# SysCV/LiDAR_snow_sim

Hardware: AMD Instinct MI355X
Metric: augmented points/s/GPU (64x2048 sweep, 2.5 mm/h); HBM roofline % -- value: rows resident in HBM when the clock starts (device-resident API: augment_batch on CUDA tensors); with H2D of the rows and D2H of the results inside the clock: value_pcie_inclusive (higher is better)
Workload: dtype f64

## Files before the change

### lidar_snow_sim_amd/csrc/sg_beam.h

```cpp
#pragma once
#include "sg_math.h"
#include "sg_atan_cr.h"
#include "sg_range_index.h"

#if defined(__HIP_DEVICE_COMPILE__)
#define SG_GLOBAL __attribute__((address_space(1)))
#else
#define SG_GLOBAL
#endif
template <typename P> __device__ __forceinline__ const SG_GLOBAL P *sg_gptr(const P *p) { return (const SG_GLOBAL P *)p; }

#if defined(__HIP_DEVICE_COMPILE__)
template <int CTRL, int ROW_MASK> __device__ __forceinline__ int sg_dpp(int old, int v) { return __builtin_amdgcn_update_dpp(old, v, CTRL, ROW_MASK, 0xf, false); }
__device__ __forceinline__ int sg_wave_incl_add(int v)
{
    v += sg_dpp<0x111, 0xf>(0, v); v += sg_dpp<0x112, 0xf>(0, v); v += sg_dpp<0x114, 0xf>(0, v); v += sg_dpp<0x118, 0xf>(0, v);
    v += sg_dpp<0x142, 0xa>(0, v);
    v += sg_dpp<0x143, 0xc>(0, v);
    return v;
}
__device__ __forceinline__ int sg_wave_incl_max(int v)
{
    constexpr int I = (int)0x80000000;
    v = max(v, sg_dpp<0x111, 0xf>(I, v)); v = max(v, sg_dpp<0x112, 0xf>(I, v)); v = max(v, sg_dpp<0x114, 0xf>(I, v)); v = max(v, sg_dpp<0x118, 0xf>(I, v));
// ... 261 lines not shown
typedef unsigned int SgTailRaw __attribute__((ext_vector_type(4)));
__device__ __forceinline__ SgTailRaw sg_tail_load(const SG_GLOBAL SgEntry *fp) { return *reinterpret_cast<const SG_GLOBAL SgTailRaw *>(&fp->rho); }
__device__ __forceinline__ SgTail sg_tail_pin(SgTailRaw v)
{
    asm volatile("" : "+v"(v));
    SgTail t; t.rho = __hiloint2double((int)v.y, (int)v.x); t.flags = v.z;
    return t;
}
#else
typedef SgTail SgTailRaw;
__device__ __forceinline__ SgTailRaw sg_tail_load(const SgEntry *fp) { SgTail t; t.rho = fp->rho; t.flags = fp->flags; return t; }
__device__ __forceinline__ SgTail sg_tail_pin(SgTailRaw v) { return v; }
#endif

__device__ __forceinline__ uint32_t sg_hit_word(uint32_t e, bool hit_r, bool hit_l)
{
    return e | (hit_r ? 0x40000000u : 0u) | (hit_l ? 0x80000000u : 0u);
}
__device__ __forceinline__ void sg_hit_angles(uint32_t w, const SgEntry *__restrict__ entries, double theta_r, double theta_l, double &a1, double &a2)
{
    const SG_GLOBAL SgEntry *f = sg_gptr(entries) + (w & 0x3fffffffu);
    a1 = (w & 0x40000000u) ? theta_r : f->t0;
    a2 = (w & 0x80000000u) ? theta_l : f->t1;
}

template <int N>
__device__ __forceinline__ void sg_hit_angles_all(const uint32_t (&w)[N], int L, const SgEntry *__restrict__ entries, double theta_r, double theta_l,
                                                  double (&a1)[N], double (&a2)[N])
{
#if defined(__HIP_DEVICE_COMPILE__)
    SgTailRaw raw[N];
#pragma unroll
    for (int j = 0; j < N; ++j) {
        const SG_GLOBAL SgEntry *f = sg_gptr(entries) + (j < L ? (w[j] & 0x3fffffffu) : 0u);
        raw[j] = *reinterpret_cast<const SG_GLOBAL SgTailRaw *>(&f->t0);
    }
#pragma unroll
    for (int j = 0; j < N; ++j) {
        a1[j] = (w[j] & 0x40000000u) ? theta_r : __hiloint2double((int)raw[j].y, (int)raw[j].x);
        a2[j] = (w[j] & 0x80000000u) ? theta_l : __hiloint2double((int)raw[j].w, (int)raw[j].z);
    }
#else
    for (int j = 0; j < N; ++j) if (j < L) sg_hit_angles(w[j], entries, theta_r, theta_l, a1[j], a2[j]);
#endif
}

struct SgQsPair { uint32_t x, y; };
#if defined(__HIP_DEVICE_COMPILE__)
typedef unsigned int SgQsRaw __attribute__((ext_vector_type(2), aligned(4)));
__device__ __forceinline__ SgQsPair sg_qs_load(const SG_GLOBAL uint32_t *p)
{
    const SgQsRaw v = *reinterpret_cast<const SG_GLOBAL SgQsRaw *>(p);
    return SgQsPair{v.x, v.y};
}
#else
__device__ __forceinline__ SgQsPair sg_qs_load(const uint32_t *p) { return SgQsPair{p[0], p[1]}; }
#endif

template <typename T, int LMAX, int STRIDE, bool DEFER = false, bool COMPACT = false, bool UTAB = false>
__device__ __forceinline__ int sg_wave_scan_t(bool act, T px, T py, T pz, const SgTable tab, double beam_div_deg, double *s_a1, double *s_a2,
                                              double *s_rho, int *s_cnt, int *s_key, int *s_st, int tid, SgBeamOut &out, T &d_t, T &theta_t,
                                              bool EXACT_TAN, double *ov_blk = nullptr, int ov_cap = 0)
{
    out.overflow = 0; out.range_error = 0; out.diff2 = 0.0; out.has_power = 0; out.n_flakes = 0; out.n_hits = 0;
    out.label = 0; out.new_i = 0; out.k_best = 0;
    const int lane = tid & 63, wbase = tid & ~63;
    SgBeamGeo g{};
// ... 718 lines not shown
```

### lidar_snow_sim_amd/csrc/sg_common.h

```cpp
#pragma once
#include <stddef.h>
#include <stdint.h>

#define SG_PI 3.141592653589793
#define SG_TWO_PI (2 * SG_PI)
#define SG_RBINS 1230
#define SG_NBINS 2048
#define SG_BIN_MARGIN 1e-6
#define SG_BEAM_MARGIN 1e-9
#define SG_TBL_STRIDE 16
#define SG_BLKREC 8
#define SG_HITS_UNDECIDED 0x40000000
#define SG_MAX_LASERS 256
#define SG_LCAP 63
#define SG_TILE 1024

struct SgEntry {
    double phi;
    double x, y, r;
    double t0, t1;
    double rho;
    uint32_t flags;
    uint32_t src;
};
// ... 54 lines not shown
    const SgLasers *las;
    const double *rgrid;
    double beam_div_deg;
    uint32_t *rec;
    uint32_t *rec_q;
    void *rng;
    int32_t *status;
    int32_t *tier_hint;
    unsigned long long *diff2;
    int32_t exact_math;
    int32_t n_cls;
    int32_t cls_cap[SG_MAX_CLASSES];
    const int32_t *seg_blk;
    const int64_t *seg_start;
    const int32_t *seg_cnt;
    const int32_t *seg_frame;
    const int32_t *seg_n;
    const int32_t *seg_of_blk;
    int64_t grid_blocks;
    int32_t q_chunk;
    int64_t blk_lo, blk_hi;
    const int32_t *chunk_blk;
    int32_t chunk;
    double *dq;
    int32_t *dq_g;
    uint16_t *dq_sc;
    unsigned long long *qn;
    int2_t *pw_items;
    int32_t *pw_count;
    int2_t *pw_items1;
    int32_t front_max;
    int64_t n_regions_ub;
    int32_t blk_rows;
    int32_t kp_lds_quarters;
    int64_t dq_n;
    int32_t *tier_list;
    int32_t *tier_info;
    int64_t tier_stride;
    int32_t *tier_sparse;
    int32_t *tn, *tbase;
    int32_t cls;
    int32_t work_lo, work_hi;
    int32_t work_hint;
    int32_t *redo_list;
    int32_t *redo_cnt;
    double *tq;
    uint16_t *tq_sc;
// ... 126 lines not shown
```

### lidar_snow_sim_amd/csrc/sg_host.h

```cpp
#pragma once
#include <hip/hip_runtime.h>

#include <algorithm>
#include <array>
#include <cmath>
#include <cstdio>
#include <cstdlib>
#include <cstring>
#include <string>
#include <vector>

#include "../../include/snowgpu.h"
#include "sg_common.h"
#include "sg_prepass.h"
#include "sg_plane.h"
#include "sg_assemble.h"
#include "sg_device_args.h"

#pragma GCC visibility push(hidden)

struct DeviceTable {
    SgEntry *entries = nullptr;
    uint32_t *bin_start = nullptr;
    uint32_t *bin_q = nullptr;
// ... 59 lines not shown
    DevBuf<int32_t> fpss_tile, fpss_seg;
    DevBuf<uint32_t> ball_entry, ball_cell;
    DevBuf<uint8_t> ball_x, ball_y, ball_z;
    DevBuf<int32_t> ball_src;
    DevBuf<unsigned long long> range_key;
    DevBuf<uint32_t> nn_entry;
    DevBuf<int32_t> nn_box;
    DevBuf<uint8_t> nn_rec;
    DevBuf<double> box_rec;
    DevBuf<unsigned long long> box_table;
    DevBuf<double> roi_rec;
    DevBuf<unsigned long long> roi_table;
    DevBuf<int32_t> roi_runs;
    DevBuf<double> iou_rec;
    DevBuf<int32_t> nms_order, nms_cand;
    DevBuf<int32_t> tile_hist, tile_base, perm, ctile_cnt, ctile_base, table_ids, out_src;
    DevBuf<uint8_t> srows;
    DevBuf<int32_t> tile_unsorted, frame_unsorted;
    DevBuf<unsigned long long> seg_tbl_cnt, seg_tbl_base;
    DevBuf<int32_t> seg_blk, seg_cnt, seg_frame, seg_n, seg_of_blk;
    DevBuf<int64_t> seg_start;
    DevBuf<uint32_t> rec, rec_q;
    DevBuf<uint8_t> rng;
    DevBuf<double> dq;
    DevBuf<int32_t> dq_g;
    DevBuf<uint16_t> dq_sc;
    DevBuf<unsigned long long> qn;
    DevBuf<int2_t> pw_items;
    DevBuf<double> ov;
    DevBuf<uint16_t> ov_sc;
    DevBuf<int32_t> tier_list, tier_sparse, tbase, redo_list;
    DevBuf<double> tq[SG_MAX_CLASSES];
    DevBuf<uint16_t> tq_sc[SG_MAX_CLASSES];
    DevBuf<double> h_lists;
    int64_t tier_cap_override = 0;
    int first_tier_override = 0;
    int few = 2;
    int heavy_tail = -1;
    int tier_rows = -1;
    hipStream_t lane_stream[3] = {nullptr, nullptr, nullptr};
    int stats_early = -1;
    int prepass_with_few = -1;
    bool serial = false;
    DevBuf<int32_t> chunk_blk;
    DevBuf<uint16_t> rank;
    DevBuf<uint8_t> keep, rows_in, rows_out;
    DevBuf<int64_t> frame_off, out_counts, out_stats;
// ... 166 lines not shown
```

### lidar_snow_sim_amd/csrc/snowgpu_batch.cpp

```cpp
#include "sg_host.h"
#include "sg_launch.h"

static int sync_tables(snowgpu_ctx *ctx)
{
    if (!ctx->tables_dirty) return SNOWGPU_OK;
    const size_t n = std::max<size_t>(ctx->tables.size(), 1);
    if (n > ctx->d_tables_cap) {
        if (ctx->d_tables) { (void)hipStreamSynchronize(ctx->stream); (void)hipFree(ctx->d_tables); }
        HIPCHK(ctx, hipMalloc((void **)&ctx->d_tables, n * sizeof(SgTable)));
        ctx->d_tables_cap = n;
    }
    std::vector<SgTable> h(n);
    for (size_t i = 0; i < ctx->tables.size(); ++i) h[i] = ctx->tables[i].desc;
    HIPCHK(ctx, hipMemcpy(ctx->d_tables, h.data(), n * sizeof(SgTable), hipMemcpyHostToDevice));
    ctx->tables_dirty = false;
    return SNOWGPU_OK;
}

static void choose_tiers(const snowgpu_ctx *ctx, double beam_div_deg, int tiers[4], int *n_tiers)
{
    const double expect = (double)ctx->max_flakes * (beam_div_deg * (SG_PI / 180.0)) / SG_TWO_PI;
    int first = expect <= 24.0 ? 4 : (expect <= 48.0 ? 8 : (expect <= 96.0 ? 16 : SG_LCAP));
    if (ctx->first_tier_override == 4 || ctx->first_tier_override == 8 || ctx->first_tier_override == 16 ||
        ctx->first_tier_override == SG_LCAP)
// ... 190 lines not shown
    const int h_lanes = 256;
    const int h_cap = (int)std::min<uint32_t>(std::max<uint32_t>(R->max_flakes, 64u), 8192u);
    a.n_cls = n_cls;
    for (int k = 0; k + 1 < n_cls; ++k) a.cls_cap[k] = tiers[k + 1];
    a.cls_cap[n_cls - 1] = h_cap;
    ENSURE(ctx, ctx->h_lists, (size_t)4 * (size_t)(h_cap + 1) * (size_t)h_lanes);
    a.h_lists = ctx->h_lists.p; a.h_cap = h_cap; a.h_lanes = h_lanes;
    a.tier_list = ctx->tier_list.p; a.tier_stride = b.n_total; a.tier_sparse = ctx->tier_sparse.p;
    if (tier_rows) {
        ENSURE(ctx, ctx->redo_list, n * (size_t)n_tiers);
        a.redo_list = ctx->redo_list.p;
    }
    const bool use_ov = tiers[0] < SG_OV_CAP && n_cls >= 2 && !tier_rows &&
                        R->tier_cap_override <= 0 && n * SG_OV_STRIDE * sizeof(double) <= ((size_t)40 << 30);
    int64_t tq_caps[SG_MAX_CLASSES] = {0, 0, 0, 0};
    for (int k = 0; k + 1 < n_cls && !tier_rows; ++k) {
        if (use_ov && tiers[k + 1] <= SG_OV_CAP) continue;
        tq_caps[k] = tier_queue_cap(R, tiers[k + 1], b.n_total);
        ENSURE(ctx, ctx->tq[k], ((size_t)tq_caps[k] + 64) * (3 * (size_t)tiers[k + 1] + 2));
        ENSURE(ctx, ctx->tq_sc[k], (size_t)tq_caps[k]);
    }
    a.q_chunk = (int32_t)q_chunk;
    {
        const size_t planes = 3 * (size_t)tiers[0] + 2;
        if (n * planes * sizeof(double) > ((size_t)64 << 30))
            return fail(ctx, SNOWGPU_E_INVALID, "batch too large for the dict queue of this table density: split it");
        if (b.n_frames >= (1 << 22)) return fail(ctx, SNOWGPU_E_INVALID, "too many frames in one batch");
        ENSURE(ctx, ctx->dq, (n + 64) * planes);
        ENSURE(ctx, ctx->dq_g, n);
        ENSURE(ctx, ctx->dq_sc, n);
        if (!seg_small) HIPCHK(ctx, hipMemsetAsync(ctx->qn.p, 0, sizeof(unsigned long long) * zero_words, st));
        a.tn = (int32_t *)(ctx->qn.p + regions); a.tbase = ctx->tbase.p;
        a.diff2 = ctx->qn.p + 3 * regions;
        int32_t *small = (int32_t *)(ctx->qn.p + 3 * regions + (size_t)b.n_frames);
        a.tier_info = small; a.pw_count = small + 8; a.redo_cnt = small + 12;
        a.dq = ctx->dq.p; a.dq_g = ctx->dq_g.p; a.dq_sc = ctx->dq_sc.p; a.qn = ctx->qn.p; a.dq_n = b.n_total;
        const int lanes = first_block < 64 ? first_block : 64;
        a.n_regions_ub = use_seg ? (int64_t)b.n_frames * 256 : (b.n_total + a.q_chunk - 1) / a.q_chunk;
        a.blk_rows = first_block;
        a.kp_lds_quarters = 2;
        const size_t items_cap = n / (size_t)lanes + 2 * (size_t)a.n_regions_ub + 64;
        ENSURE(ctx, ctx->pw_items, 2 * items_cap);
        a.pw_items = ctx->pw_items.p;
        a.pw_items1 = (R->few > 0 && !b.dbg_count && lanes == 64) ? ctx->pw_items.p + items_cap : nullptr;
        a.front_max = a.pw_items1 ? std::min(R->few, std::min(3, tiers[0])) : 1;
    }
    if (use_ov) {
        ENSURE(ctx, ctx->ov, (n + 256) * SG_OV_STRIDE);
        ENSURE(ctx, ctx->ov_sc, n + 256);
        a.ov = ctx->ov.p; a.ov_sc = ctx->ov_sc.p; a.ov_cap = SG_OV_CAP;
    }
// ... 171 lines not shown
```

### lidar_snow_sim_amd/csrc/snowgpu_kernels.hip

```cpp
#include <hip/hip_runtime.h>
#include <algorithm>
#include "sg_beam.h"
#include "sg_few.h"
#include "sg_kutil.h"
#include "sg_launch.h"

#ifndef SG_NB4
#define SG_NB4 4
#endif
#ifndef SG_KP_WIN
#define SG_KP_WIN 3
#endif
#ifndef SG_FP_WAVES
#define SG_FP_WAVES 6
#endif
#ifndef SG_FP_WAVES_SEG
#define SG_FP_WAVES_SEG 7
#endif
#ifndef SG_NB_TIERS
#define SG_NB_TIERS 4
#endif
#ifndef SG_KP_THREE_MAX
#define SG_KP_THREE_MAX 16
#endif
#ifndef SG_KP_THREE_MIN
#define SG_KP_THREE_MIN 8
// ... 205 lines not shown
            } else {
                tier_k = k;
                pending = true;
            }
        } else if (o.range_error) {
            atomicCAS(&a.status[0], 0, 4 );
            atomicCAS(&a.status[1], -1, (int32_t)g);
        }
    }
    if constexpr (!LIST) {
        if (__ballot(tier_k >= 0)) {
            for (int k = 0; k < a.n_cls; ++k) {
                const unsigned long long m = __ballot(tier_k == k);
                if (!m) continue;
                const int leader = __ffsll((long long)m) - 1;
                int base = 0;
                if ((tid & 63) == leader) base = atomicAdd(&a.tn[(int64_t)__builtin_amdgcn_readfirstlane(region) * SG_MAX_CLASSES + k], (int)__popcll(m));
                base = __shfl(base, leader);
                if (tier_k == k) a.tier_sparse[(int64_t)k * a.tier_stride + q_base + base + (int)__popcll(m & sg_lanemask_lt())] = (int32_t)g;
            }
        }
    }
    if constexpr (DICT) {
        constexpr int P = SG_QPLANES(LMAX);
        auto hand_over = [&](double *q, int64_t slot) {
            q[sg_qaddr<P>(slot, 0)] = (double)d_t;
            q[sg_qaddr<P>(slot, 1)] = (double)theta_t;
            double th_r, th_l;
            sg_beam_limits((double)theta_t, a.beam_div_deg, th_r, th_l);
            if constexpr (LMAX <= 4) {
                double x1[LMAX], x2[LMAX];
                uint32_t hw[LMAX];
#pragma unroll
                for (int j = 0; j < LMAX; ++j) hw[j] = reinterpret_cast<const uint32_t *>(s_a1)[j * BLOCK + tid];
                sg_hit_angles_all<LMAX>(hw, L, tab.entries, th_r, th_l, x1, x2);
#pragma unroll
                for (int j = 0; j < LMAX; ++j)
                    if (j < L) {
                        q[sg_qaddr<P>(slot, 2 + 3 * j)] = x1[j];
                        q[sg_qaddr<P>(slot, 3 + 3 * j)] = x2[j];
                        q[sg_qaddr<P>(slot, 4 + 3 * j)] = s_rho[j * BLOCK + tid];
                    }
            } else {
                for (int j = 0; j < L; ++j) {
                    double x1, x2;
                    sg_hit_angles(reinterpret_cast<const uint32_t *>(s_a1)[j * BLOCK + tid], tab.entries, th_r, th_l, x1, x2);
                    q[sg_qaddr<P>(slot, 2 + 3 * j)] = x1;
                    q[sg_qaddr<P>(slot, 3 + 3 * j)] = x2;
                    q[sg_qaddr<P>(slot, 4 + 3 * j)] = s_rho[j * BLOCK + tid];
                }
            }
        };
        const bool front = o.has_power && L <= a.front_max, back = o.has_power && L > a.front_max;
        const unsigned long long mf = __ballot(front), mb = __ballot(back);
        if (mf | mb) {
            const int leader = __ffsll((long long)(mf | mb)) - 1;
            unsigned long long base = 0;
            if ((tid & 63) == leader)
                base = atomicAdd(&a.qn[__builtin_amdgcn_readfirstlane(region)], (unsigned long long)__popcll(mf) | ((unsigned long long)__popcll(mb) << 32));
            const unsigned blo = __shfl((unsigned)(base & 0xffffffffull), leader), bhi = __shfl((unsigned)(base >> 32), leader);
            if (o.has_power) {
                const int64_t slot = front ? q_base + (int)blo + (int)__popcll(mf & sg_lanemask_lt())
                                           : q_base + q_size - 1 - ((int)bhi + (int)__popcll(mb & sg_lanemask_lt()));
                hand_over(a.dq, slot);
                a.dq_g[slot] = (int32_t)g;
                a.dq_sc[slot] = (uint16_t)(L | (ch << 8));
                rec = SG_REC_SLOT | (uint32_t)slot;
            }
        }
    } else {
        constexpr int NB = LMAX <= 4 ? 4 : 8;
        if (o.has_power) {
            double best = 0.0;
// ... 138 lines not shown
    }
    for (int k = 0; k < nb; k += lanes_back)
        a.pw_items[base++] = make_int2((int)(q_base + q_size - nb + k), (nb - k < lanes_back ? nb - k : lanes_back) | (f1 << 10));
}

__global__ __launch_bounds__(256) void k_tier_gather(SgBeamArgs a, int n_regions_ub)
{
    const int r = blockIdx.x * 4 + (int)(threadIdx.x >> 6), lane = (int)(threadIdx.x & 63);
    if (blockIdx.x == 0 && threadIdx.x < SG_MAX_CLASSES) a.status[2 + threadIdx.x] = a.tier_info[threadIdx.x];
    if (blockIdx.x == 0 && threadIdx.x < SG_MAX_CLASSES && a.tier_hint) a.tier_hint[threadIdx.x] = a.tier_info[threadIdx.x];
    if (blockIdx.x == 0 && threadIdx.x == 0 && a.tier_hint) a.tier_hint[SG_MAX_CLASSES] = (int32_t)((a.n_total >> 10) + 1);
    int q_size = 0, f1 = 0;
    int64_t q_base = 0;
    if (!sg_region(a, r, n_regions_ub, q_base, q_size, f1)) return;
    for (int k = 0; k < a.n_cls; ++k) {
        const int c = a.tn[(int64_t)r * SG_MAX_CLASSES + k];
        if (c == 0) continue;
        const int32_t *src = a.tier_sparse + (int64_t)k * a.tier_stride + q_base;
        int32_t *dst = a.tier_list + (int64_t)k * a.tier_stride + a.tbase[(int64_t)r * SG_MAX_CLASSES + k];
        for (int i = lane; i < c; i += 64) dst[i] = src[i];
    }
}

template <typename T, int LMAX, int BLOCK, bool LISTQ>
__device__ __forceinline__ void sg_kp_item(const SgBeamArgs &a, char *smem, const int ov_list, const int64_t work_off,
                                           const int start, const int cnt, const int item_f)
{
    constexpr int LANES = BLOCK < 64 ? BLOCK : 64;
    constexpr int WIN = BLOCK < 64 ? 1 : SG_KP_WIN;
    constexpr int P = SG_QPLANES(LMAX);
    double *s_a1 = (double *)smem;
    constexpr bool THREE = SG_KP_THREE_MAX > 0 && LMAX <= SG_KP_THREE_MAX && LMAX >= SG_KP_THREE_MIN;
    double *s_a2 = s_a1 + (LMAX + 1) * BLOCK;
    double *s_rho = s_a2 + (LMAX + 1) * BLOCK;
    double *s_ratio = THREE ? s_rho : s_rho + (LMAX + 1) * BLOCK;
    double *s_work = THREE ? s_a2 : s_ratio;
    const int tid = threadIdx.x, lane = tid & 63;
    const int ltid = BLOCK < 64 ? lane : tid;
    const double *planes = LISTQ ? a.tq : a.dq;
    const uint16_t *scs = LISTQ ? a.tq_sc : a.dq_sc;
    static_assert(WIN <= 4, "the window's permutation passes through one 64-double row segment of the wave");
    uint16_t *s_perm = (uint16_t *)(s_ratio + (BLOCK < 64 ? 0 : (tid & ~63)));
    int perm[WIN];
    const bool sorted = WIN > 1 && cnt > LANES;
    if constexpr (WIN > 1) {
        if (sorted) {
            int key[WIN], rank[WIN];
            int64_t at[WIN];
            unsigned scw[WIN];
#pragma unroll
            for (int r = 0; r < WIN; ++r) { const int idx = r * 64 + lane; at[r] = (int64_t)start + (idx < cnt ? idx : 0); }
            if (LISTQ && ov_list) {
#pragma unroll
                for (int r = 0; r < WIN; ++r) at[r] = (int64_t)a.tier_list[work_off + at[r]];
#pragma unroll
                for (int r = 0; r < WIN; ++r) scw[r] = (unsigned)a.ov_sc[at[r]];
            } else {
#pragma unroll
                for (int r = 0; r < WIN; ++r) scw[r] = (unsigned)scs[at[r]];
            }
#pragma unroll
            for (int r = 0; r < WIN; ++r) {
// ... 15 lines not shown
            place(254); place(255);
#pragma unroll
            for (int r = 0; r < WIN; ++r) s_perm[rank[r]] = (uint16_t)(r * 64 + lane);
            asm volatile("s_waitcnt lgkmcnt(0)" ::: "memory");
#pragma unroll
            for (int r = 0; r < WIN; ++r) perm[r] = s_perm[r * 64 + lane];
            asm volatile("s_waitcnt lgkmcnt(0)" ::: "memory");
        }
    }
    const int rounds = (cnt + LANES - 1) / LANES;
    for (int r = 0; r < rounds; ++r) {
        const int idx = r * LANES + lane;
        const bool in = lane < LANES && idx < cnt;
        int pos = idx;
        if constexpr (WIN > 1) {
            if (sorted) {
#pragma unroll
                for (int q = 0; q < WIN; ++q) if (q == r) pos = perm[q];
            }
        }
        const int64_t slot = (int64_t)start + pos;
        unsigned sc = 0xffffu;
        int32_t g = 0;
        double d = 0.0, tc = 0.0, f_a1 = 0.0, f_a2 = 0.0, f_rho = 0.0;
        const double *qb = planes;
        int qs = 64;
        if (in) {
            g = LISTQ ? a.tier_list[work_off + slot] : a.dq_g[slot];
            if (LISTQ && ov_list) { qb = a.ov + (size_t)g * SG_OV_STRIDE; qs = 1; sc = a.ov_sc[g]; }
            else { qb = planes + sg_qaddr<P>(slot, 0); sc = scs[slot]; }
            d = qb[0];
            tc = qb[qs];
            f_a1 = qb[2 * qs]; f_a2 = qb[3 * qs]; f_rho = qb[4 * qs];
        }
        const bool live = in && sc != 0xffffu;
        const int L = (int)(sc & 255u), ch = (int)(sc >> 8);
        int f = 0;
        SgBeamOut o;
        o.overflow = 0; o.range_error = 0; o.diff2 = 0.0; o.has_power = 0; o.n_flakes = 0; o.n_hits = 0; o.label = 0; o.new_i = 0; o.k_best = 0;
        constexpr int NB = LMAX <= 4 ? SG_NB4 : SG_NB_TIERS;
        int S = 0, nw = 0, k_best = 0;
        double best = 0.0;
        if (live) {
            f = item_f >= 0 ? item_f : sg_frame_of(a, g);
            unsigned long long ord = 0xfedcba9876543210ull;
            if (LISTQ) {
                s_a1[ltid] = f_a1; s_a2[ltid] = f_a2; s_rho[ltid] = f_rho;
                if constexpr (THREE) ord = 0;
                for (int h0 = 1; h0 < L; h0 += 8) {
                    double xa[8], xb[8], xr[8];
#pragma unroll
                    for (int c = 0; c < 8; ++c) {
                        const int h = h0 + c < L ? h0 + c : 0;
                        xa[c] = qb[(2 + 3 * h) * qs]; xb[c] = qb[(3 + 3 * h) * qs]; xr[c] = qb[(4 + 3 * h) * qs];
                    }
#pragma unroll
                    for (int c = 0; c < 8; ++c)
                        if (h0 + c < L) { s_a1[(h0 + c) * BLOCK + ltid] = xa[c]; s_a2[(h0 + c) * BLOCK + ltid] = xb[c]; s_rho[(h0 + c) * BLOCK + ltid] = xr[c]; }
                }
                for (int h = 1; h < L; ++h) {
                    const double x1 = s_a1[h * BLOCK + ltid], x2 = s_a2[h * BLOCK + ltid], r = s_rho[h * BLOCK + ltid];
                    int q = h;
                    while (q > 0 && (s_rho[(q - 1) * BLOCK + ltid] > r ||
                                     (s_rho[(q - 1) * BLOCK + ltid] == r && ov_list &&
                                      (s_a1[(q - 1) * BLOCK + ltid] > x1 || (s_a1[(q - 1) * BLOCK + ltid] == x1 && s_a2[(q - 1) * BLOCK + ltid] > x2))))) {
                        s_rho[q * BLOCK + ltid] = s_rho[(q - 1) * BLOCK + ltid]; s_a1[q * BLOCK + ltid] = s_a1[(q - 1) * BLOCK + ltid];
                        s_a2[q * BLOCK + ltid] = s_a2[(q - 1) * BLOCK + ltid];
                        --q;
                    }
                    if (q != h) { s_rho[q * BLOCK + ltid] = r; s_a1[q * BLOCK + ltid] = x1; s_a2[q * BLOCK + ltid] = x2; }
                    if constexpr (THREE) {
                        const unsigned long long low = (1ull << (4 * q)) - 1ull;
                        ord = (ord & low) | ((unsigned long long)h << (4 * q)) | ((ord & ~low) << 4);
                    }
                }
            } else {
                s_a1[ltid] = f_a1; s_a2[ltid] = f_a2;
                if constexpr (!THREE) s_rho[ltid] = f_rho;
                if constexpr (LMAX <= 4 && !THREE) {
                    double xa[LMAX - 1], xb[LMAX - 1], xr[LMAX - 1];
#pragma unroll
                    for (int j = 1; j < LMAX; ++j) { xa[j - 1] = qb[(2 + 3 * j) * qs]; xb[j - 1] = qb[(3 + 3 * j) * qs]; xr[j - 1] = qb[(4 + 3 * j) * qs]; }
#pragma unroll
                    for (int j = 1; j < LMAX; ++j)
                        if (j < L) { s_a1[j * BLOCK + ltid] = xa[j - 1]; s_a2[j * BLOCK + ltid] = xb[j - 1]; s_rho[j * BLOCK + ltid] = xr[j - 1]; }
                } else {
                    for (int j = 1; j < L; ++j) {
                        s_a1[j * BLOCK + ltid] = qb[(2 + 3 * j) * qs];
                        s_a2[j * BLOCK + ltid] = qb[(3 + 3 * j) * qs];
                        if constexpr (!THREE) s_rho[j * BLOCK + ltid] = qb[(4 + 3 * j) * qs];
                    }
                }
            }
            auto queue_rho = [&](int j) -> double {
                const int h = (int)((ord >> (4 * j)) & 15ull);
                return h == 0 ? f_rho : qb[(4 + 3 * h) * qs];
            };
            int32_t *dc = a.dbg_count ? a.dbg_count + g : nullptr;
            double *drj = a.dbg_count ? a.dbg_rj + (int64_t)g * a.dbg_cap : nullptr;
            double *dra = a.dbg_count ? a.dbg_ratio + (int64_t)g * a.dbg_cap : nullptr;
            unsigned long long srcmap = 0;
            if constexpr (THREE) S = sg_beam_dict<LMAX, BLOCK, false>(L, tc, d, a.beam_div_deg, s_a1, s_a2, nullptr, s_ratio, ltid, 0, nullptr, nullptr, nullptr, 0, &srcmap);
            else S = sg_beam_dict<LMAX, BLOCK>(L, tc, d, a.beam_div_deg, s_a1, s_a2, s_rho, s_ratio, ltid, a.dbg_cap, dc, drj, dra);
            if constexpr (THREE) {
                if (dc) {
                    *dc = S + 1;
                    for (int t = 0; t <= S && t < a.dbg_cap; ++t) {
                        const int j = (int)((srcmap >> (4 * t)) & 15ull);
                        drj[t] = t == S ? d : queue_rho(j);
                        dra[t] = s_ratio[t * BLOCK + ltid];
                    }
                }
            }
            if (S > 0) {
                const T d_t = (T)d;
                if constexpr (THREE) {
                    sg_beam_amp3<T, LMAX, BLOCK>(d_t, S, ch, a.las, s_a1, s_a2, s_rho, ltid, o,
                                                 [&](int t) { return queue_rho((int)((srcmap >> (4 * t)) & 15ull)); });
                } else sg_beam_amp<T, LMAX, BLOCK>(d_t, S, ch, a.las, s_a1, s_a2, s_rho, s_ratio, ltid, o, 0);
// ... 40 lines not shown
        if (work_n > a.work_hi) work_n = a.work_hi;
        work_off = (int64_t)a.cls * a.tier_stride;
        if (WIN > 1 && work_n <= (int64_t)step * LANES) item_slots = LANES;
        n_items = (int)((work_n + item_slots - 1) / item_slots);
    } else {
        n_items = *a.pw_count;
    }
    for (int i = (int)blockIdx.x * WAVES + __builtin_amdgcn_readfirstlane(tid >> 6); i < n_items; i += step) {
        int start, cnt, item_f = -1;
        if (LISTQ) {
            start = i * item_slots;
            cnt = (int)(work_n - start < item_slots ? work_n - start : item_slots);
        } else {
            const int2 d = a.pw_items[i];
            start = __builtin_amdgcn_readfirstlane(d.x);
            const int dy = __builtin_amdgcn_readfirstlane(d.y);
            cnt = dy & 1023; item_f = (dy >> 10) - 1;
        }
        sg_kp_item<T, LMAX, BLOCK, LISTQ>(a, smem, a.ov_list, work_off, start, cnt, item_f);
    }
}

template <typename T, int N>
__global__ __launch_bounds__(256, 4) void k_power_few(SgBeamArgs a, int qplanes)
{
    __shared__ double s_amp[N + 1][256], s_rho[N + 1][256], s_best[256];
    __shared__ int s_win[N + 1][256], s_zone[N + 1][256], s_k[256];
    __shared__ int s_mark[256];
    const int tid = (int)threadIdx.x, lane = tid & 63, wbase = tid & ~63;
    const int n_items = a.pw_count[1];
    const int step = (int)gridDim.x * 4;
    for (int i = (int)blockIdx.x * 4 + __builtin_amdgcn_readfirstlane(tid >> 6); i < n_items; i += step) {
        const int2 it = a.pw_items1[i];
        const int start = __builtin_amdgcn_readfirstlane(it.x), dy = __builtin_amdgcn_readfirstlane(it.y);
        const int cnt = dy & 1023, item_f = (dy >> 10) - 1;
        const bool live = lane < cnt;
        const int64_t slot = (int64_t)start + lane;
        SgBeamOut o;
        o.overflow = 0; o.range_error = 0; o.diff2 = 0.0; o.has_power = 0; o.n_flakes = 0; o.n_hits = 0; o.label = 0; o.new_i = 0; o.k_best = 0;
        int f = 0, ch = 0, S = 0, g = 0;
        SgFew<N> P{};
        int zone[N + 1], n = 0;
#pragma unroll
        for (int z = 0; z <= N; ++z) zone[z] = 0;
        if (live) {
            const double *q = a.dq + (slot >> 6) * (int64_t)(qplanes * 64) + (slot & 63);
            const unsigned sc = a.dq_sc[slot];
            const double d = q[0], tc = q[64];
            double a1[N], a2[N], rho[N];
#pragma unroll
            for (int j = 0; j < N; ++j) {
                a1[j] = q[(2 + 3 * j) * 64]; a2[j] = q[(3 + 3 * j) * 64]; rho[j] = q[(4 + 3 * j) * 64];
            }
            ch = (int)(sc >> 8);
            g = a.dq_g[slot];
            f = item_f >= 0 ? item_f : sg_frame_of(a, g);
            S = sg_few_prep<T, N>(d, tc, (int)(sc & 255u), a1, a2, rho, ch, a.las, a.beam_div_deg, P, o);
            if (S) {
                int ka, kb;
                sg_few_zone<N, 0>(P, 0.0, ka, kb);
                if (kb >= ka) { zone[0] = ka | ((kb - ka + 1) << 16); n += kb - ka + 1; }
                if constexpr (N >= 2) { sg_few_zone<N, 1>(P, 0.0, ka, kb); if (kb >= ka) { zone[1] = ka | ((kb - ka + 1) << 16); n += kb - ka + 1; } }
                if constexpr (N >= 3) { sg_few_zone<N, 2>(P, 0.0, ka, kb); if (kb >= ka) { zone[2] = ka | ((kb - ka + 1) << 16); n += kb - ka + 1; } }
                sg_few_zone<N, N>(P, 0.0, ka, kb);
                if (kb >= ka) { zone[N] = ka | ((kb - ka + 1) << 16); n += kb - ka + 1; }
            }
        }
#pragma unroll
        for (int t = 0; t < N; ++t) { s_amp[t][tid] = P.amp[t]; s_rho[t][tid] = P.rho[t]; s_win[t][tid] = P.k0[t] | (P.k1[t] << 16); }
        s_amp[N][tid] = P.tamp; s_rho[N][tid] = P.d; s_win[N][tid] = P.tk0 | (P.tk1 << 16);
#pragma unroll
        for (int z = 0; z <= N; ++z) s_zone[z][tid] = zone[z];
        s_best[tid] = 0.0; s_k[tid] = 0;
        asm volatile("" ::: "memory");
        const int incl = sg_wave_incl_add(n);
        const int excl = incl - n;
        const int total = __builtin_amdgcn_readlane(incl, 63);
        for (int base = 0; base < total; base += 64) {
            const int p = base + lane;
// ... 155 lines not shown
    constexpr int THREADS = BLOCK < 64 ? 64 : BLOCK, LANES = BLOCK < 64 ? BLOCK : 64;
    const int cus = sg_cu_count();
    unsigned per_cu = (unsigned)std::min<size_t>(32 * 64 / THREADS, std::max<size_t>(1, (size_t)(160 * 1024) / lds));
    if (!LISTQ && a->kp_lds_quarters > 0 && a->kp_lds_quarters < 4) per_cu = std::max(1u, per_cu * (unsigned)a->kp_lds_quarters / 4u);
    int64_t blocks = (int64_t)cus * per_cu;
    int64_t items_ub = LISTQ ? ((int64_t)a->work_hi + LANES - 1) / LANES : (a->n_total + LANES - 1) / LANES + 2 * a->n_regions_ub;
    if (LISTQ && a->work_hint > 0) items_ub = std::min<int64_t>(items_ub, (4 * (int64_t)a->work_hint + LANES - 1) / LANES + 8);
    blocks = std::min<int64_t>(blocks, (items_ub + THREADS / 64 - 1) / (THREADS / 64));
    if (blocks <= 0) return 0;
    if (!LISTQ) {
        const unsigned pg = (unsigned)((a->n_regions_ub + 255) / 256);
        if (pg == 0) return 0;
        const int64_t back_est = a->n_total / 10;
        const int lanes_back = (BLOCK < 64 || back_est <= (int64_t)blocks * (THREADS / 64) * LANES * 5 / 2) ? LANES : LANES * SG_KP_WIN;
        if (plan_only) {
            hipLaunchKernelGGL(k_power_plan, dim3(pg), dim3(256), 0, st, *a, LANES, lanes_back, (int)a->n_regions_ub);
            SG_CHECK_LAUNCH();
            return 0;
        }
        if (a->pw_items1 && (which & 1)) {
            hipStream_t s1 = st;
            const unsigned g1 = (unsigned)std::min<int64_t>((int64_t)cus * 4, (a->n_total / LANES + a->n_regions_ub + 3) / 4);
            if (g1 > 0) {
                if (a->front_max == 1) hipLaunchKernelGGL((k_power_few<T, 1>), dim3(g1), dim3(256), 0, s1, *a, SG_QPLANES(LMAX));
                else if (a->front_max == 2) hipLaunchKernelGGL((k_power_few<T, 2>), dim3(g1), dim3(256), 0, s1, *a, SG_QPLANES(LMAX));
                else hipLaunchKernelGGL((k_power_few<T, 3>), dim3(g1), dim3(256), 0, s1, *a, SG_QPLANES(LMAX));
            }
            SG_CHECK_LAUNCH();
            if (ev_few && hipEventRecord(ev_few, st) != hipSuccess) return (int)hipGetLastError();
        }
    }
    if (!(which & 2)) return 0;
    hipLaunchKernelGGL((k_power<T, LMAX, BLOCK, LISTQ>), dim3((unsigned)blocks), dim3(THREADS), lds, st, *a);
    SG_CHECK_LAUNCH();
    return 0;
}

extern "C" int sg_launch_tier_scan(const SgBeamArgs *a, int dtype, int lmax, void *stream)
{
    const int64_t n = (int64_t)a->work_hi - a->work_lo;
    if (n <= 0) return 0;
    int64_t want = (n + 255) / 256;
    if (a->work_hint > 0) want = std::min<int64_t>(want, (4 * (int64_t)a->work_hint + 255) / 256 + 8);
    const unsigned blocks = (unsigned)std::min<int64_t>(want, (int64_t)sg_cu_count() * 8);
    return sg_by_dtype_tier<false>(dtype, lmax, [&](auto t, auto tier) {
        hipLaunchKernelGGL((k_tier_scan_direct<decltype(t), decltype(tier)::LMAX>), dim3(blocks), dim3(256), 0, (hipStream_t)stream, *a);
        SG_CHECK_LAUNCH();
        return 0;
    });
// ... 54 lines not shown
```

Before: 10.08 billion.

## Store compact entry indices in the dict queue and resolve angles at consumer

The dict queue between the beam scan and the power kernels now holds a 32-bit entry word per hit plus a header (float or double d/theta), instead of three doubles (a1, a2, rho) per hit. Consumers (k_power non-list path and k_power_few) recompute beam limits and gather t0/t1/rho from the per-frame entry table. This cuts queue write and read traffic and the queue footprint. The cost is an extra dependent gather from the entry table on the consumer side. For f32 the header is stored as float, which lowers d/theta precision in the queue.

```diff
diff --git a/lidar_snow_sim_amd/csrc/sg_beam.h b/lidar_snow_sim_amd/csrc/sg_beam.h
--- a/lidar_snow_sim_amd/csrc/sg_beam.h
+++ b/lidar_snow_sim_amd/csrc/sg_beam.h
@@ -307,27 +307,6 @@
     const SG_GLOBAL SgEntry *f = sg_gptr(entries) + (w & 0x3fffffffu);
     a1 = (w & 0x40000000u) ? theta_r : f->t0;
     a2 = (w & 0x80000000u) ? theta_l : f->t1;
-}
-
-template <int N>
-__device__ __forceinline__ void sg_hit_angles_all(const uint32_t (&w)[N], int L, const SgEntry *__restrict__ entries, double theta_r, double theta_l,
-                                                  double (&a1)[N], double (&a2)[N])
-{
-#if defined(__HIP_DEVICE_COMPILE__)
-    SgTailRaw raw[N];
-#pragma unroll
-    for (int j = 0; j < N; ++j) {
-        const SG_GLOBAL SgEntry *f = sg_gptr(entries) + (j < L ? (w[j] & 0x3fffffffu) : 0u);
-        raw[j] = *reinterpret_cast<const SG_GLOBAL SgTailRaw *>(&f->t0);
-    }
-#pragma unroll
-    for (int j = 0; j < N; ++j) {
-        a1[j] = (w[j] & 0x40000000u) ? theta_r : __hiloint2double((int)raw[j].y, (int)raw[j].x);
-        a2[j] = (w[j] & 0x80000000u) ? theta_l : __hiloint2double((int)raw[j].w, (int)raw[j].z);
-    }
-#else
-    for (int j = 0; j < N; ++j) if (j < L) sg_hit_angles(w[j], entries, theta_r, theta_l, a1[j], a2[j]);
-#endif
 }
 
 struct SgQsPair { uint32_t x, y; };
diff --git a/lidar_snow_sim_amd/csrc/sg_common.h b/lidar_snow_sim_amd/csrc/sg_common.h
--- a/lidar_snow_sim_amd/csrc/sg_common.h
+++ b/lidar_snow_sim_amd/csrc/sg_common.h
@@ -100,7 +100,7 @@
     int64_t blk_lo, blk_hi;
     const int32_t *chunk_blk;
     int32_t chunk;
-    double *dq;
+    uint32_t *dq;
     int32_t *dq_g;
     uint16_t *dq_sc;
     unsigned long long *qn;
diff --git a/lidar_snow_sim_amd/csrc/sg_host.h b/lidar_snow_sim_amd/csrc/sg_host.h
--- a/lidar_snow_sim_amd/csrc/sg_host.h
+++ b/lidar_snow_sim_amd/csrc/sg_host.h
@@ -105,7 +105,7 @@
     DevBuf<int64_t> seg_start;
     DevBuf<uint32_t> rec, rec_q;
     DevBuf<uint8_t> rng;
-    DevBuf<double> dq;
+    DevBuf<uint32_t> dq;
     DevBuf<int32_t> dq_g;
     DevBuf<uint16_t> dq_sc;
     DevBuf<unsigned long long> qn;
diff --git a/lidar_snow_sim_amd/csrc/sg_queue.h b/lidar_snow_sim_amd/csrc/sg_queue.h
--- /dev/null
+++ b/lidar_snow_sim_amd/csrc/sg_queue.h
@@ -0,0 +1,83 @@
+#pragma once
+#include "sg_beam.h"
+
+#ifndef SG_DQ_ROW_HEADER
+#define SG_DQ_ROW_HEADER 1
+#endif
+#if defined(__HIP_DEVICE_COMPILE__)
+#define SG_DQ_RECORD(entries, w) (sg_gptr(entries) + ((w) & 0x3fffffffu))
+#else
+#define SG_DQ_RECORD(entries, w) ((entries) + ((w) & 0x3fffffffu))
+#endif
+
+__host__ __device__ __forceinline__ constexpr int sg_dq_hdr(int elem_size) { return SG_DQ_ROW_HEADER ? elem_size / 4 : 2; }
+__host__ __device__ __forceinline__ constexpr int sg_dq_slot_words(int lmax, int hdr) { return 2 * hdr + lmax; }
+__host__ __device__ __forceinline__ int64_t sg_dq_cell(int64_t slot, int plane, int lmax, int hdr)
+{
+    const int64_t group = (slot >> 6) * (int64_t)(64 * sg_dq_slot_words(lmax, hdr));
+    const int c = (int)(slot & 63);
+    return plane < 2 ? group + (int64_t)((plane * 64 + c) * hdr) : group + (int64_t)(128 * hdr + (plane - 2) * 64 + c);
+}
+
+template <typename T>
+__host__ __device__ __forceinline__ void sg_dq_store_header(uint32_t *q, int64_t slot, int lmax, T d_t, T theta_t)
+{
+    constexpr int H = sg_dq_hdr((int)sizeof(T));
+    using S = std::conditional_t<H == 2, double, float>;
+    *reinterpret_cast<S *>(q + sg_dq_cell(slot, 0, lmax, H)) = (S)d_t;
+    *reinterpret_cast<S *>(q + sg_dq_cell(slot, 1, lmax, H)) = (S)theta_t;
+}
+template <typename T>
+__host__ __device__ __forceinline__ void sg_dq_store_word(uint32_t *q, int64_t slot, int lmax, int j, uint32_t w)
+{
+    q[sg_dq_cell(slot, 2 + j, lmax, sg_dq_hdr((int)sizeof(T)))] = w;
+}
+
+template <typename T>
+__host__ __device__ __forceinline__ void sg_dq_load_header(const uint32_t *q, int64_t slot, int lmax, double &d, double &theta_c)
+{
+    constexpr int H = sg_dq_hdr((int)sizeof(T));
+    using S = std::conditional_t<H == 2, double, float>;
+    d = (double)*reinterpret_cast<const S *>(q + sg_dq_cell(slot, 0, lmax, H));
+    theta_c = (double)*reinterpret_cast<const S *>(q + sg_dq_cell(slot, 1, lmax, H));
+}
+template <typename T>
+__host__ __device__ __forceinline__ uint32_t sg_dq_load_word(const uint32_t *q, int64_t slot, int lmax, int j)
+{
+    return q[sg_dq_cell(slot, 2 + j, lmax, sg_dq_hdr((int)sizeof(T)))];
+}
+
+__host__ __device__ __forceinline__ void sg_dq_resolve(uint32_t w, const SgEntry *__restrict__ entries, double theta_r, double theta_l, double &a1, double &a2,
+                                                       double &rho)
+{
+    const auto *f = SG_DQ_RECORD(entries, w);
+    a1 = (w & 0x40000000u) ? theta_r : f->t0;
+    a2 = (w & 0x80000000u) ? theta_l : f->t1;
+    rho = f->rho;
+}
+__host__ __device__ __forceinline__ double sg_dq_rho(uint32_t w, const SgEntry *__restrict__ entries) { return SG_DQ_RECORD(entries, w)->rho; }
+
+template <int N>
+__host__ __device__ __forceinline__ void sg_dq_resolve_all(const uint32_t (&w)[N], int L, const SgEntry *__restrict__ entries, double theta_r, double theta_l,
+                                                           double (&a1)[N], double (&a2)[N], double (&rho)[N])
+{
+#if defined(__HIP_DEVICE_COMPILE__)
+    typedef unsigned int Raw2 __attribute__((ext_vector_type(2)));
+    SgTailRaw ang[N];
+    Raw2 rng[N];
+#pragma unroll
+    for (int j = 0; j < N; ++j) {
+        const SG_GLOBAL SgEntry *f = SG_DQ_RECORD(entries, j < L ? w[j] : 0u);
+        ang[j] = *reinterpret_cast<const SG_GLOBAL SgTailRaw *>(&f->t0);
+        rng[j] = *reinterpret_cast<const SG_GLOBAL Raw2 *>(&f->rho);
+    }
+#pragma unroll
+    for (int j = 0; j < N; ++j) {
+        a1[j] = (w[j] & 0x40000000u) ? theta_r : __hiloint2double((int)ang[j].y, (int)ang[j].x);
+        a2[j] = (w[j] & 0x80000000u) ? theta_l : __hiloint2double((int)ang[j].w, (int)ang[j].z);
+        rho[j] = __hiloint2double((int)rng[j].y, (int)rng[j].x);
+    }
+#else
+    for (int j = 0; j < N; ++j) sg_dq_resolve(j < L ? w[j] : 0u, entries, theta_r, theta_l, a1[j], a2[j], rho[j]);
+#endif
+}
diff --git a/lidar_snow_sim_amd/csrc/snowgpu_batch.cpp b/lidar_snow_sim_amd/csrc/snowgpu_batch.cpp
--- a/lidar_snow_sim_amd/csrc/snowgpu_batch.cpp
+++ b/lidar_snow_sim_amd/csrc/snowgpu_batch.cpp
@@ -1,5 +1,6 @@
 #include "sg_host.h"
 #include "sg_launch.h"
+#include "sg_queue.h"
 
 static int sync_tables(snowgpu_ctx *ctx)
 {
@@ -236,11 +237,11 @@
     }
     a.q_chunk = (int32_t)q_chunk;
     {
-        const size_t planes = 3 * (size_t)tiers[0] + 2;
-        if (n * planes * sizeof(double) > ((size_t)64 << 30))
+        const size_t slot_words = (size_t)sg_dq_slot_words(tiers[0], sg_dq_hdr(b.dtype == 0 ? 4 : 8));
+        if (n * slot_words * sizeof(uint32_t) > ((size_t)64 << 30))
             return fail(ctx, SNOWGPU_E_INVALID, "batch too large for the dict queue of this table density: split it");
         if (b.n_frames >= (1 << 22)) return fail(ctx, SNOWGPU_E_INVALID, "too many frames in one batch");
-        ENSURE(ctx, ctx->dq, (n + 64) * planes);
+        ENSURE(ctx, ctx->dq, (n + 64) * slot_words);
         ENSURE(ctx, ctx->dq_g, n);
         ENSURE(ctx, ctx->dq_sc, n);
         if (!seg_small) HIPCHK(ctx, hipMemsetAsync(ctx->qn.p, 0, sizeof(unsigned long long) * zero_words, st));
diff --git a/lidar_snow_sim_amd/csrc/snowgpu_kernels.hip b/lidar_snow_sim_amd/csrc/snowgpu_kernels.hip
--- a/lidar_snow_sim_amd/csrc/snowgpu_kernels.hip
+++ b/lidar_snow_sim_amd/csrc/snowgpu_kernels.hip
@@ -2,6 +2,7 @@
 #include <algorithm>
 #include "sg_beam.h"
 #include "sg_few.h"
+#include "sg_queue.h"
 #include "sg_kutil.h"
 #include "sg_launch.h"
 
@@ -253,33 +254,15 @@
         }
     }
     if constexpr (DICT) {
-        constexpr int P = SG_QPLANES(LMAX);
-        auto hand_over = [&](double *q, int64_t slot) {
-            q[sg_qaddr<P>(slot, 0)] = (double)d_t;
-            q[sg_qaddr<P>(slot, 1)] = (double)theta_t;
-            double th_r, th_l;
-            sg_beam_limits((double)theta_t, a.beam_div_deg, th_r, th_l);
+        auto hand_over = [&](uint32_t *q, int64_t slot) {
+            sg_dq_store_header<T>(q, slot, LMAX, d_t, theta_t);
+            const uint32_t *s_w = reinterpret_cast<const uint32_t *>(s_a1);
             if constexpr (LMAX <= 4) {
-                double x1[LMAX], x2[LMAX];
-                uint32_t hw[LMAX];
-#pragma unroll
-                for (int j = 0; j < LMAX; ++j) hw[j] = reinterpret_cast<const uint32_t *>(s_a1)[j * BLOCK + tid];
-                sg_hit_angles_all<LMAX>(hw, L, tab.entries, th_r, th_l, x1, x2);
 #pragma unroll
                 for (int j = 0; j < LMAX; ++j)
-                    if (j < L) {
-                        q[sg_qaddr<P>(slot, 2 + 3 * j)] = x1[j];
-                        q[sg_qaddr<P>(slot, 3 + 3 * j)] = x2[j];
-                        q[sg_qaddr<P>(slot, 4 + 3 * j)] = s_rho[j * BLOCK + tid];
-                    }
+                    if (j < L) sg_dq_store_word<T>(q, slot, LMAX, j, s_w[j * BLOCK + tid]);
             } else {
-                for (int j = 0; j < L; ++j) {
-                    double x1, x2;
-                    sg_hit_angles(reinterpret_cast<const uint32_t *>(s_a1)[j * BLOCK + tid], tab.entries, th_r, th_l, x1, x2);
-                    q[sg_qaddr<P>(slot, 2 + 3 * j)] = x1;
-                    q[sg_qaddr<P>(slot, 3 + 3 * j)] = x2;
-                    q[sg_qaddr<P>(slot, 4 + 3 * j)] = s_rho[j * BLOCK + tid];
-                }
+                for (int j = 0; j < L; ++j) sg_dq_store_word<T>(q, slot, LMAX, j, s_w[j * BLOCK + tid]);
             }
         };
         const bool front = o.has_power && L <= a.front_max, back = o.has_power && L > a.front_max;
@@ -464,6 +447,11 @@
     }
 }
 
+__device__ __forceinline__ const SgEntry *sg_dq_entries(const SgBeamArgs &a, int f, int ch)
+{
+    return a.frame_tables[(int64_t)f * a.las->n + ch].entries;
+}
+
 template <typename T, int LMAX, int BLOCK, bool LISTQ>
 __device__ __forceinline__ void sg_kp_item(const SgBeamArgs &a, char *smem, const int ov_list, const int64_t work_off,
                                            const int start, const int cnt, const int item_f)
@@ -479,7 +467,7 @@
     double *s_work = THREE ? s_a2 : s_ratio;
     const int tid = threadIdx.x, lane = tid & 63;
     const int ltid = BLOCK < 64 ? lane : tid;
-    const double *planes = LISTQ ? a.tq : a.dq;
+    const double *planes = a.tq;
     const uint16_t *scs = LISTQ ? a.tq_sc : a.dq_sc;
     static_assert(WIN <= 4, "the window's permutation passes through one 64-double row segment of the wave");
     uint16_t *s_perm = (uint16_t *)(s_ratio + (BLOCK < 64 ? 0 : (tid & ~63)));
@@ -541,16 +529,29 @@
         const int64_t slot = (int64_t)start + pos;
         unsigned sc = 0xffffu;
         int32_t g = 0;
-        double d = 0.0, tc = 0.0, f_a1 = 0.0, f_a2 = 0.0, f_rho = 0.0;
-        const double *qb = planes;
-        int qs = 64;
+        double d = 0.0, tc = 0.0, f_rho = 0.0;
+        [[maybe_unused]] double f_a1 = 0.0, f_a2 = 0.0;
+        [[maybe_unused]] const double *qb = planes;
+        [[maybe_unused]] int qs = 64;
+        constexpr int NW = LMAX <= 4 ? LMAX : 1;
+        [[maybe_unused]] uint32_t hw[NW];
+#pragma unroll
+        for (int j = 0; j < NW; ++j) hw[j] = 0u;
         if (in) {
-            g = LISTQ ? a.tier_list[work_off + slot] : a.dq_g[slot];
-            if (LISTQ && ov_list) { qb = a.ov + (size_t)g * SG_OV_STRIDE; qs = 1; sc = a.ov_sc[g]; }
-            else { qb = planes + sg_qaddr<P>(slot, 0); sc = scs[slot]; }
-            d = qb[0];
-            tc = qb[qs];
-            f_a1 = qb[2 * qs]; f_a2 = qb[3 * qs]; f_rho = qb[4 * qs];
+            if constexpr (LISTQ) {
+                g = a.tier_list[work_off + slot];
+                if (ov_list) { qb = a.ov + (size_t)g * SG_OV_STRIDE; qs = 1; sc = a.ov_sc[g]; }
+                else { qb = planes + sg_qaddr<P>(slot, 0); sc = scs[slot]; }
+                d = qb[0];
+                tc = qb[qs];
+                f_a1 = qb[2 * qs]; f_a2 = qb[3 * qs]; f_rho = qb[4 * qs];
+            } else {
+                g = a.dq_g[slot];
+                sc = scs[slot];
+                sg_dq_load_header<T>(a.dq, slot, LMAX, d, tc);
+#pragma unroll
+                for (int j = 0; j < NW; ++j) hw[j] = sg_dq_load_word<T>(a.dq, slot, LMAX, j);
+            }
         }
         const bool live = in && sc != 0xffffu;
         const int L = (int)(sc & 255u), ch = (int)(sc >> 8);
@@ -563,7 +564,8 @@
         if (live) {
             f = item_f >= 0 ? item_f : sg_frame_of(a, g);
             unsigned long long ord = 0xfedcba9876543210ull;
-            if (LISTQ) {
+            [[maybe_unused]] const SgEntry *ent = nullptr;
+            if constexpr (LISTQ) {
                 s_a1[ltid] = f_a1; s_a2[ltid] = f_a2; s_rho[ltid] = f_rho;
                 if constexpr (THREE) ord = 0;
                 for (int h0 = 1; h0 < L; h0 += 8) {
@@ -594,26 +596,41 @@
                     }
                 }
             } else {
-                s_a1[ltid] = f_a1; s_a2[ltid] = f_a2;
-                if constexpr (!THREE) s_rho[ltid] = f_rho;
-                if constexpr (LMAX <= 4 && !THREE) {
-                    double xa[LMAX - 1], xb[LMAX - 1], xr[LMAX - 1];
-#pragma unroll
-                    for (int j = 1; j < LMAX; ++j) { xa[j - 1] = qb[(2 + 3 * j) * qs]; xb[j - 1] = qb[(3 + 3 * j) * qs]; xr[j - 1] = qb[(4 + 3 * j) * qs]; }
-#pragma unroll
-                    for (int j = 1; j < LMAX; ++j)
-                        if (j < L) { s_a1[j * BLOCK + ltid] = xa[j - 1]; s_a2[j * BLOCK + ltid] = xb[j - 1]; s_rho[j * BLOCK + ltid] = xr[j - 1]; }
+                ent = sg_dq_entries(a, f, ch);
+                double th_r, th_l;
+                sg_beam_limits(tc, a.beam_div_deg, th_r, th_l);
+                if constexpr (LMAX <= 4) {
+                    double xa[LMAX], xb[LMAX], xr[LMAX];
+                    sg_dq_resolve_all<LMAX>(hw, L, ent, th_r, th_l, xa, xb, xr);
+                    f_rho = xr[0];
+#pragma unroll
+                    for (int j = 0; j < LMAX; ++j)
+                        if (j < L) {
+                            s_a1[j * BLOCK + ltid] = xa[j]; s_a2[j * BLOCK + ltid] = xb[j];
+                            if constexpr (!THREE) s_rho[j * BLOCK + ltid] = xr[j];
+                        }
                 } else {
-                    for (int j = 1; j < L; ++j) {
-                        s_a1[j * BLOCK + ltid] = qb[(2 + 3 * j) * qs];
-                        s_a2[j * BLOCK + ltid] = qb[(3 + 3 * j) * qs];
-                        if constexpr (!THREE) s_rho[j * BLOCK + ltid] = qb[(4 + 3 * j) * qs];
+                    for (int j0 = 0; j0 < L; j0 += 8) {
+                        uint32_t w8[8];
+                        double xa[8], xb[8], xr[8];
+                        w8[0] = j0 == 0 ? hw[0] : sg_dq_load_word<T>(a.dq, slot, LMAX, j0);
+#pragma unroll
+                        for (int c = 1; c < 8; ++c) w8[c] = sg_dq_load_word<T>(a.dq, slot, LMAX, j0 + c < L ? j0 + c : 0);
+                        sg_dq_resolve_all<8>(w8, L - j0, ent, th_r, th_l, xa, xb, xr);
+                        if (j0 == 0) f_rho = xr[0];
+#pragma unroll
+                        for (int c = 0; c < 8; ++c)
+                            if (j0 + c < L) {
+                                s_a1[(j0 + c) * BLOCK + ltid] = xa[c]; s_a2[(j0 + c) * BLOCK + ltid] = xb[c];
+                                if constexpr (!THREE) s_rho[(j0 + c) * BLOCK + ltid] = xr[c];
+                            }
                     }
                 }
             }
             auto queue_rho = [&](int j) -> double {
                 const int h = (int)((ord >> (4 * j)) & 15ull);
-                return h == 0 ? f_rho : qb[(4 + 3 * h) * qs];
+                if constexpr (LISTQ) return h == 0 ? f_rho : qb[(4 + 3 * h) * qs];
+                else return h == 0 ? f_rho : sg_dq_rho(sg_dq_load_word<T>(a.dq, slot, LMAX, h), ent);
             };
             int32_t *dc = a.dbg_count ? a.dbg_count + g : nullptr;
             double *drj = a.dbg_count ? a.dbg_rj + (int64_t)g * a.dbg_cap : nullptr;
@@ -700,7 +717,7 @@
 }
 
 template <typename T, int N>
-__global__ __launch_bounds__(256, 4) void k_power_few(SgBeamArgs a, int qplanes)
+__global__ __launch_bounds__(256, 4) void k_power_few(SgBeamArgs a, int lmax)
 {
     __shared__ double s_amp[N + 1][256], s_rho[N + 1][256], s_best[256];
     __shared__ int s_win[N + 1][256], s_zone[N + 1][256], s_k[256];
@@ -722,17 +739,19 @@
 #pragma unroll
         for (int z = 0; z <= N; ++z) zone[z] = 0;
         if (live) {
-            const double *q = a.dq + (slot >> 6) * (int64_t)(qplanes * 64) + (slot & 63);
             const unsigned sc = a.dq_sc[slot];
-            const double d = q[0], tc = q[64];
-            double a1[N], a2[N], rho[N];
-#pragma unroll
-            for (int j = 0; j < N; ++j) {
-                a1[j] = q[(2 + 3 * j) * 64]; a2[j] = q[(3 + 3 * j) * 64]; rho[j] = q[(4 + 3 * j) * 64];
-            }
+            double d, tc;
+            sg_dq_load_header<T>(a.dq, slot, lmax, d, tc);
+            uint32_t w[N];
+#pragma unroll
+            for (int j = 0; j < N; ++j) w[j] = sg_dq_load_word<T>(a.dq, slot, lmax, j);
             ch = (int)(sc >> 8);
             g = a.dq_g[slot];
             f = item_f >= 0 ? item_f : sg_frame_of(a, g);
+            const SgEntry *ent = sg_dq_entries(a, f, ch);
+            double th_r, th_l, a1[N], a2[N], rho[N];
+            sg_beam_limits(tc, a.beam_div_deg, th_r, th_l);
+            sg_dq_resolve_all<N>(w, (int)(sc & 255u), ent, th_r, th_l, a1, a2, rho);
             S = sg_few_prep<T, N>(d, tc, (int)(sc & 255u), a1, a2, rho, ch, a.las, a.beam_div_deg, P, o);
             if (S) {
                 int ka, kb;
@@ -934,9 +953,9 @@
             hipStream_t s1 = st;
             const unsigned g1 = (unsigned)std::min<int64_t>((int64_t)cus * 4, (a->n_total / LANES + a->n_regions_ub + 3) / 4);
             if (g1 > 0) {
-                if (a->front_max == 1) hipLaunchKernelGGL((k_power_few<T, 1>), dim3(g1), dim3(256), 0, s1, *a, SG_QPLANES(LMAX));
-                else if (a->front_max == 2) hipLaunchKernelGGL((k_power_few<T, 2>), dim3(g1), dim3(256), 0, s1, *a, SG_QPLANES(LMAX));
-                else hipLaunchKernelGGL((k_power_few<T, 3>), dim3(g1), dim3(256), 0, s1, *a, SG_QPLANES(LMAX));
+                if (a->front_max == 1) hipLaunchKernelGGL((k_power_few<T, 1>), dim3(g1), dim3(256), 0, s1, *a, LMAX);
+                else if (a->front_max == 2) hipLaunchKernelGGL((k_power_few<T, 2>), dim3(g1), dim3(256), 0, s1, *a, LMAX);
+                else hipLaunchKernelGGL((k_power_few<T, 3>), dim3(g1), dim3(256), 0, s1, *a, LMAX);
             }
             SG_CHECK_LAUNCH();
             if (ev_few && hipEventRecord(ev_few, st) != hipSuccess) return (int)hipGetLastError();
```

Result: faster. 10.43 billion, median of 6 (+3.5%).
